# matchylabs/matchy

Measured on AMD Instinct MI355X. Metric: log GB/s scanned (matchy match hot path, 100K IoCs), higher is better.
Workload: dtype u8

## Files before the change

include/matchy_amd.h:

```cpp
#ifndef MATCHY_AMD_H
#define MATCHY_AMD_H

#include <stdbool.h>
#include <stddef.h>
#include <stdint.h>

#ifdef __cplusplus
extern "C" {
#endif

#define MATCHY_SUCCESS 0
#define MATCHY_ERROR_FILE_NOT_FOUND -1
#define MATCHY_ERROR_INVALID_FORMAT -2
#define MATCHY_ERROR_CORRUPT_DATA -3
#define MATCHY_ERROR_OUT_OF_MEMORY -4
#define MATCHY_ERROR_INVALID_PARAM -5
#define MATCHY_ERROR_IO -6

#define MATCHY_EXTRACT_DOMAINS (1 << 0)
#define MATCHY_EXTRACT_EMAILS (1 << 1)
#define MATCHY_EXTRACT_IPV4 (1 << 2)
#define MATCHY_EXTRACT_IPV6 (1 << 3)
#define MATCHY_EXTRACT_HASHES (1 << 4)
#define MATCHY_EXTRACT_BITCOIN (1 << 5)
// ... 290 lines not shown
typedef struct matchy_gz_piece_t {
    uint64_t start_bit, end_bit;
    uint32_t member;
    uint32_t produced, out_pos;
    uint32_t flags;
} matchy_gz_piece_t;
#define MATCHY_PIECE_HAS_START 1u
#define MATCHY_PIECE_LIVE 2u
#define MATCHY_PIECE_HANDED_OVER 4u
int32_t matchy_scanner_set_gz_pieces(matchy_scanner_t *scanner, uint32_t piece_bytes);
uint32_t matchy_scanner_get_gz_pieces(const matchy_scanner_t *scanner);
int32_t matchy_scan_result_gz_pieces(const matchy_scan_result_t *result, const matchy_gz_piece_t **pieces, size_t *n, const uint32_t **first_piece);
void matchy_scanner_get_gz_pieces_timing(const matchy_scanner_t *scanner, float out_ms[6]);
typedef struct matchy_gz_stream_state_t { uint64_t text_bytes; uint32_t crc, bit, history_len; uint8_t history[32768]; } matchy_gz_stream_state_t;
typedef struct matchy_gz_stream_window_t {
    const matchy_gz_stream_state_t *state;
    const uint8_t *carry; uint32_t carry_len, carry_cap, text_cap, flags;
} matchy_gz_stream_window_t;
#define MATCHY_STREAM_FIRST 1u
#define MATCHY_STREAM_FILE_END 2u
#define MATCHY_STREAM_OK 0
#define MATCHY_STREAM_NO_LINE_END 1
#define MATCHY_STREAM_NO_PROGRESS 2
#define MATCHY_STREAM_FAILED 3
int32_t matchy_scanner_scan_gz_stream(matchy_scanner_t *scanner, const uint8_t *packed, size_t packed_len, const matchy_gz_stream_window_t *window,
                                      uint32_t fetch_mode, bool want_text, matchy_scan_result_t *result);
int32_t matchy_scan_result_gz_stream(const matchy_scan_result_t *result, int32_t *status, int32_t *gz_status, uint64_t *consumed_bits, uint32_t *text_len,
                                     bool *ended, const matchy_gz_stream_state_t **state_out, const uint8_t **carry, size_t *carry_len);
#define MATCHY_STREAM_PASSES 8
void matchy_scanner_get_gz_stream_timing(const matchy_scanner_t *scanner, float out_ms[MATCHY_STREAM_PASSES]);
void matchy_scanner_set_profile(matchy_scanner_t *scanner, bool enabled);
void matchy_scanner_set_slices(matchy_scanner_t *scanner, int32_t slices);
int32_t matchy_scanner_last_slices(const matchy_scanner_t *scanner);
void matchy_scanner_get_timing(const matchy_scanner_t *scanner, float out_ms[5]);
char *matchy_amd_query_json(const matchy_t *db, const char *query, int32_t *found);
matchy_extractor_t *matchy_amd_extractor_create(uint32_t flags, uint32_t min_domain_labels);
void matchy_amd_extractor_set_unique(matchy_extractor_t *extractor, bool enabled);
bool matchy_amd_extractor_unique(const matchy_extractor_t *extractor);
void matchy_amd_extractor_reset_unique(matchy_extractor_t *extractor);
uint64_t matchy_amd_extractor_unique_count(const matchy_extractor_t *extractor);
const char *matchy_amd_last_error(void);
int32_t matchy_amd_ac_dfa_states(const matchy_t *db);
int32_t matchy_amd_suffix_filter(const matchy_t *db);
void *matchy_amd_pinned_alloc(size_t bytes);
void matchy_amd_pinned_free(void *ptr);
int32_t matchy_amd_host_register(const void *ptr, size_t bytes);
void matchy_amd_host_unregister(const void *ptr);
int32_t matchy_amd_device_count(void);
int32_t matchy_amd_device_numa_node(int32_t device);
int32_t matchy_amd_bind_thread_to_device(int32_t device);
int32_t matchy_amd_unbind_thread(void);
int32_t matchy_amd_numa_cpus(const char *sysfs_root, const char *pci_bus_id, int32_t *out_cpus, size_t cap);

typedef struct matchy_multi_scanner_t matchy_multi_scanner_t;
typedef struct matchy_multi_batch_t {
  size_t seq;
  int32_t status;
  matchy_scan_result_t result;
  const uint8_t *data;
  size_t len;
  void *tag;
  void *payload;
  size_t worker;
} matchy_multi_batch_t;
typedef struct matchy_multi_totals_t { uint64_t batches, bytes, lines, candidates, matches; } matchy_multi_totals_t;
typedef void *(*matchy_multi_batch_fn)(void *user, size_t worker, matchy_scanner_t *scanner, const matchy_scan_result_t *result,
// ... 66 lines not shown
```

matchy_amd/__init__.py:

```python
import ctypes as C
import os
import json
from pathlib import Path

from . import build as _build

__all__ = ["DatabaseBuilder", "Database", "Extractor", "Scanner", "lib", "ITEM_TYPE_NAMES", "EXTRACT_ALL", "last_error"]

PKG = Path(__file__).resolve().parent
LIB_PATH = PKG / "lib" / "libmatchy_amd.so"

ITEM_TYPE_NAMES = ["Domain", "Email", "IPv4", "IPv6", "MD5", "SHA1", "SHA256", "SHA384", "SHA512", "Bitcoin", "Ethereum", "Monero"]
EXTRACT_DOMAINS, EXTRACT_EMAILS, EXTRACT_IPV4, EXTRACT_IPV6 = 1, 2, 4, 8
EXTRACT_HASHES, EXTRACT_BITCOIN, EXTRACT_ETHEREUM, EXTRACT_MONERO = 16, 32, 64, 128
EXTRACT_ALL = 255

EXPORTED_SYMBOLS = [
    "matchy_builder_new", "matchy_builder_set_case_insensitive", "matchy_builder_add", "matchy_builder_set_description",
    "matchy_builder_save", "matchy_builder_build", "matchy_builder_free", "matchy_init_open_options",
    "matchy_open_with_options", "matchy_open", "matchy_open_buffer", "matchy_close", "matchy_query", "matchy_query_into",
    "matchy_free_result", "matchy_free_string", "matchy_result_to_json", "matchy_version", "matchy_format",
    "matchy_has_ip_data", "matchy_has_string_data", "matchy_has_literal_data", "matchy_has_glob_data", "matchy_metadata",
    "matchy_get_pattern_string", "matchy_pattern_count", "matchy_extractor_create", "matchy_extractor_extract_chunk",
    "matchy_matches_free", "matchy_extractor_free", "matchy_item_type_name", "matchy_scanner_create", "matchy_scanner_free",
    "matchy_scanner_scan", "matchy_scanner_scan_device", "matchy_scan_result_free", "matchy_scan_hit_to_json",
    "matchy_scanner_set_profile", "matchy_scanner_get_timing", "matchy_amd_last_error", "matchy_builder_set_build_epoch",
    "matchy_get_stats", "matchy_clear_cache", "matchy_has_pattern_data", "matchy_result_get_entry", "matchy_aget_value",
    "matchy_get_entry_data_list", "matchy_free_entry_data_list", "matchy_validate", "matchy_builder_set_schema",
    "matchy_amd_query_json", "matchy_amd_extractor_create", "matchy_amd_device_count", "matchy_scanner_submit_device",
    "matchy_scanner_wait", "matchy_scanner_set_slices", "matchy_scanner_last_slices", "matchy_scan_result_on_device",
    "matchy_amd_ac_dfa_states", "matchy_amd_suffix_filter", "matchy_amd_pinned_alloc", "matchy_amd_pinned_free",
    "matchy_amd_host_register", "matchy_amd_host_unregister",
    "matchy_amd_device_numa_node", "matchy_amd_bind_thread_to_device", "matchy_amd_numa_cpus",
    "matchy_multi_scanner_create", "matchy_multi_scanner_free", "matchy_multi_scanner_workers", "matchy_multi_scanner_worker_scanner",
    "matchy_multi_scanner_set_batch_hook", "matchy_multi_scanner_submit", "matchy_multi_scanner_next", "matchy_multi_scanner_scan",
    "matchy_multi_scanner_pending", "matchy_multi_scanner_max_pending", "matchy_multi_scanner_submit_near", "matchy_multi_scanner_worker_numa",
    "matchy_amd_unbind_thread",
    "matchy_multi_scanner_scan_file", "matchy_scan_result_to_ndjson",
    "matchy_scanner_set_line_context", "matchy_scanner_line_context", "matchy_scan_result_lines", "matchy_multi_scanner_set_line_context",
    "matchy_scan_result_to_ndjson_lines", "matchy_scanner_get_line_timing",
    "matchy_amd_extractor_set_unique", "matchy_amd_extractor_unique", "matchy_amd_extractor_reset_unique", "matchy_amd_extractor_unique_count",
    "matchy_scanner_set_tally", "matchy_scanner_tally", "matchy_scanner_reset_tally", "matchy_scanner_tally_top",
    "matchy_multi_scanner_set_tally", "matchy_multi_scanner_tally_top", "matchy_multi_scanner_reset_tally", "matchy_tally_free",
    "matchy_scanner_set_segments", "matchy_scan_result_segments", "matchy_scan_result_to_ndjson_segments",
    "matchy_multi_scanner_submit_segments", "matchy_scanner_get_segment_timing",
    "matchy_scanner_scan_gz", "matchy_scan_result_gz", "matchy_scanner_get_gz_timing", "matchy_multi_scanner_submit_gz",
    "matchy_scanner_scan_gz_files", "matchy_scan_result_gz_files", "matchy_multi_scanner_submit_gz_files",
    "matchy_scanner_scan_gz_window", "matchy_scan_result_gz_window", "matchy_multi_scanner_submit_gz_window", "matchy_scanner_get_gz_window_timing",
    "matchy_scanner_set_gz_pieces", "matchy_scanner_get_gz_pieces", "matchy_scan_result_gz_pieces", "matchy_scanner_get_gz_pieces_timing",
    "matchy_multi_scanner_set_gz_pieces",
    "matchy_scanner_scan_gz_stream", "matchy_scan_result_gz_stream", "matchy_scanner_get_gz_stream_timing", "matchy_multi_scanner_submit_gz_stream",
    "matchy_scanner_set_hit_lines", "matchy_scanner_hit_lines", "matchy_scan_result_hit_lines", "matchy_scanner_get_hit_lines_timing",
    "matchy_multi_scanner_set_hit_lines",
    "matchy_scanner_set_render", "matchy_scan_result_ndjson", "matchy_scanner_get_render_timing", "matchy_scanner_get_render_counters",
    "matchy_multi_scanner_set_render",
    "matchy_scanner_set_whole_lines", "matchy_scanner_whole_lines", "matchy_scanner_get_whole_lines_counters",
    "matchy_scanner_get_whole_lines_timing", "matchy_multi_scanner_set_whole_lines",
    "matchy_scanner_scan_utf16", "matchy_scan_result_utf16", "matchy_scanner_get_utf16_timing", "matchy_amd_utf16_geometry",
    "matchy_multi_scanner_submit_utf16",
]

UTF16_LE, UTF16_BE = 0, 1

# ... 224 lines not shown
        "matchy_has_literal_data": (C.c_bool, [vp]),
        "matchy_has_glob_data": (C.c_bool, [vp]),
        "matchy_metadata": (vp, [vp]),
        "matchy_get_pattern_string": (vp, [vp, C.c_uint32]),
        "matchy_pattern_count": (C.c_size_t, [vp]),
        "matchy_extractor_create": (vp, [C.c_uint32]),
        "matchy_amd_extractor_create": (vp, [C.c_uint32, C.c_uint32]),
        "matchy_extractor_extract_chunk": (C.c_int32, [vp, cp, C.c_size_t, C.POINTER(_Matches)]),
        "matchy_matches_free": (None, [C.POINTER(_Matches)]),
        "matchy_extractor_free": (None, [vp]),
        "matchy_amd_extractor_set_unique": (None, [vp, C.c_bool]),
        "matchy_amd_extractor_unique": (C.c_bool, [vp]),
        "matchy_amd_extractor_reset_unique": (None, [vp]),
        "matchy_amd_extractor_unique_count": (C.c_uint64, [vp]),
        "matchy_item_type_name": (cp, [C.c_uint8]),
        "matchy_scanner_create": (vp, [vp, C.c_uint32, C.c_int32]),
        "matchy_scanner_free": (None, [vp]),
        "matchy_scanner_scan": (C.c_int32, [vp, vp, C.c_size_t, C.POINTER(_ScanResult)]),
        "matchy_scanner_scan_device": (C.c_int32, [vp, vp, C.c_size_t, vp, C.c_uint32, C.POINTER(_ScanResult)]),
        "matchy_scanner_submit_device": (C.c_int32, [vp, vp, C.c_size_t, vp, C.c_uint32]),
        "matchy_scanner_wait": (C.c_int32, [vp, C.POINTER(_ScanResult)]),
        "matchy_scan_result_free": (None, [C.POINTER(_ScanResult)]),
        "matchy_scan_hit_to_json": (vp, [vp, C.POINTER(_ScanResult), C.c_size_t, cp, cp]),
        "matchy_scan_result_to_ndjson": (C.c_int32, [vp, C.POINTER(_ScanResult), cp, cp, C.POINTER(vp), C.POINTER(C.c_size_t)]),
        "matchy_scanner_set_profile": (None, [vp, C.c_bool]),
        "matchy_amd_ac_dfa_states": (C.c_int32, [vp]),
        "matchy_amd_suffix_filter": (C.c_int32, [vp]),
        "matchy_amd_pinned_alloc": (vp, [C.c_size_t]),
        "matchy_amd_pinned_free": (None, [vp]),
        "matchy_amd_host_register": (C.c_int32, [vp, C.c_size_t]),
        "matchy_amd_host_unregister": (None, [vp]),
        "matchy_scanner_set_slices": (None, [vp, C.c_int32]),
        "matchy_scanner_last_slices": (C.c_int32, [vp]),
        "matchy_scan_result_on_device": (C.c_bool, [C.POINTER(_ScanResult)]),
        "matchy_scanner_get_timing": (None, [vp, C.POINTER(C.c_float)]),
        "matchy_amd_last_error": (cp, []),
        "matchy_get_stats": (None, [vp, C.POINTER(_Stats)]),
        "matchy_clear_cache": (None, [vp]),
        "matchy_has_pattern_data": (C.c_bool, [vp]),
        "matchy_result_get_entry": (C.c_int32, [C.POINTER(_Result), C.POINTER(_Entry)]),
        "matchy_aget_value": (C.c_int32, [C.POINTER(_Entry), C.POINTER(_EntryData), C.POINTER(cp)]),
        "matchy_get_entry_data_list": (C.c_int32, [C.POINTER(_Entry), C.POINTER(C.POINTER(_EntryDataList))]),
        "matchy_free_entry_data_list": (None, [C.POINTER(_EntryDataList)]),
        "matchy_validate": (C.c_int32, [cp, C.c_int32, C.POINTER(vp)]),
        "matchy_builder_set_schema": (C.c_int32, [vp, cp]),
        "matchy_amd_device_count": (C.c_int32, []),
        "matchy_amd_device_numa_node": (C.c_int32, [C.c_int32]),
        "matchy_amd_bind_thread_to_device": (C.c_int32, [C.c_int32]),
        "matchy_amd_numa_cpus": (C.c_int32, [cp, cp, C.POINTER(C.c_int32), C.c_size_t]),
        "matchy_multi_scanner_create": (vp, [vp, C.c_uint32, C.POINTER(C.c_int32), C.c_size_t]),
        "matchy_multi_scanner_free": (None, [vp]),
        "matchy_multi_scanner_workers": (C.c_size_t, [vp]),
        "matchy_multi_scanner_worker_scanner": (vp, [vp, C.c_size_t]),
        "matchy_multi_scanner_submit": (C.c_int32, [vp, vp, C.c_size_t, vp, vp]),
        "matchy_multi_scanner_next": (C.c_int32, [vp, C.POINTER(_MultiBatch)]),
        "matchy_multi_scanner_submit_near": (C.c_int32, [vp, vp, C.c_size_t, vp, vp, C.c_int32]),
        "matchy_multi_scanner_worker_numa": (C.c_int32, [vp, C.c_size_t, C.POINTER(C.c_int32), C.POINTER(C.c_int32)]),
        "matchy_multi_scanner_pending": (C.c_size_t, [vp]),
        "matchy_multi_scanner_max_pending": (C.c_size_t, [vp]),
        "matchy_amd_unbind_thread": (C.c_int32, []),
        "matchy_multi_scanner_scan": (C.c_int32, [vp, vp, C.c_size_t, C.c_size_t, C.POINTER(_ScanResult)]),
        "matchy_multi_scanner_scan_file": (C.c_int32, [vp, cp, C.c_size_t, _MULTI_ORDERED_FN, vp, C.POINTER(_MultiTotals)]),
        "matchy_scanner_set_line_context": (None, [vp, C.c_bool]),
        "matchy_scanner_line_context": (C.c_bool, [vp]),
        "matchy_scan_result_lines": (C.c_int32, [C.POINTER(_ScanResult), C.POINTER(vp), C.POINTER(vp), C.POINTER(C.c_uint64)]),
        "matchy_multi_scanner_set_line_context": (None, [vp, C.c_bool]),
# ... 810 lines not shown
    def gz_pieces_timing_ms(self):
        out = (C.c_float * 6)()
        lib().matchy_scanner_get_gz_pieces_timing(self._h, out)
        return dict(find=out[0], count=out[1], chain=out[2], symbols=out[3], resolve=out[4], handover=out[5])

    def gz_window_timing_ms(self):
        out = (C.c_float * 4)()
        lib().matchy_scanner_get_gz_window_timing(self._h, out)
        return dict(inflate=out[0], crc=out[1], seal=out[2], tail=out[3])

    def gz_timing_ms(self):
        out = (C.c_float * 3)()
        lib().matchy_scanner_get_gz_timing(self._h, out)
        return dict(inflate=out[0], crc=out[1], seal=out[2])

    def set_tally(self, on=True):
        lib().matchy_scanner_set_tally(self._h, bool(on))

    def tally_enabled(self) -> bool:
        return bool(lib().matchy_scanner_tally(self._h))

    def reset_tally(self):
        lib().matchy_scanner_reset_tally(self._h)

    def tally(self, limit=0):
        return _read_tally(lib().matchy_scanner_tally_top, self._h, limit, "matchy_scanner_tally_top")

    def set_slices(self, n: int):
        lib().matchy_scanner_set_slices(self._h, n)

    def last_slices(self) -> int:
        return lib().matchy_scanner_last_slices(self._h)

    def timing_ms(self):
        out = (C.c_float * 5)()
        lib().matchy_scanner_get_timing(self._h, out)
        return dict(anchor=out[0], validate=out[1], rare=out[2], lookup=out[3], total=out[4])

    def close(self):
        if self._h:
            lib().matchy_scanner_free(self._h)
            self._h = None

    def __del__(self):
        try:
            self.close()
        except Exception:
            pass


def _gz_pack(blobs, out_lens=None):
    table = (_GzMember * len(blobs))()
    pos = 0
    for i, b in enumerate(blobs):
        table[i].offset, table[i].len = pos, len(b)
        table[i].out_len = int(out_lens[i]) if out_lens is not None and out_lens[i] else 0
        pos += len(b)
    return b"".join(bytes(b) for b in blobs), table


def _gz_pack_files(blobs):
    table = (_GzFile * len(blobs))()
    pos = 0
    for i, b in enumerate(blobs):
        table[i].offset, table[i].len = pos, len(b)
        pos += len(b)
# ... 208 lines not shown
```

matchy_amd/csrc/capi.cpp:

```cpp
#include "../../include/matchy_amd.h"

#include <algorithm>
#include <atomic>
#include <cstddef>
#include <cstdio>
#include <cstdlib>
#include <chrono>
#include <cstring>
#include <list>
#include <memory>
#include <mutex>
#include <string>
#include <unordered_map>
#include <unordered_set>
#include <vector>

#include "capi_internal.h"
#include "db_builder.h"
#include "db_image.h"
#include "engine.h"
#include "gz_stream.h"
#include "host_lookup.h"
#include "inflate_core.h"
#include "ndjson_host.h"
// ... 888 lines not shown
        for (size_t i = 0; i < in->items.size(); ++i) in->items[i].value = in->values[i].c_str();
        out->items = in->items.data(); out->count = in->items.size(); out->_internal = in;
        return MATCHY_SUCCESS;
    } catch (const HipError& ex) { set_error(ex.what); return MATCHY_ERROR_IO; }
    catch (const std::exception& ex) { set_error(ex.what()); return MATCHY_ERROR_IO; }
}
void matchy_matches_free(matchy_matches_t* m) {
    if (!m) return;
    delete reinterpret_cast<MatchesInternal*>(m->_internal);
    m->items = nullptr; m->count = 0; m->_internal = nullptr;
}

matchy_scanner_t* matchy_scanner_create(const matchy_t* dbc, uint32_t extract_flags, int32_t device) {
    if (!dbc || device < 0) return nullptr;
    Db* db = const_cast<Db*>(reinterpret_cast<const Db*>(dbc));
    try {
        if (extract_flags == 0) {
            if (db->img->has_ip) extract_flags |= EX_IPV4 | EX_IPV6;
            if (db->img->has_literal || db->img->has_glob) extract_flags |= EX_DOMAINS | EX_EMAILS | EX_HASHES | EX_BITCOIN | EX_ETHEREUM | EX_MONERO;
        }
        std::shared_ptr<DeviceDb> ddb;
        { std::lock_guard<std::mutex> lk(db->mu); ddb = db->device_db(device); }
        auto s = std::make_unique<ScannerH>();
        s->db = db;
        s->sc = std::make_unique<Scanner>(db->img, ddb, extract_flags, 2);
        return reinterpret_cast<matchy_scanner_t*>(s.release());
    } catch (const HipError& e) { set_error(e.what); return nullptr; }
    catch (const std::exception& e) { set_error(e.what()); return nullptr; }
}
void matchy_scanner_free(matchy_scanner_t* s) { delete reinterpret_cast<ScannerH*>(s); }
void matchy_scanner_set_profile(matchy_scanner_t* s, bool on) { if (s) reinterpret_cast<ScannerH*>(s)->sc->set_profile(on); }
void matchy_scanner_set_slices(matchy_scanner_t* s, int32_t n) { if (s) reinterpret_cast<ScannerH*>(s)->sc->set_slices(n); }
int32_t matchy_scanner_last_slices(const matchy_scanner_t* s) { return s ? reinterpret_cast<const ScannerH*>(s)->sc->last_slice_count() : 0; }
void matchy_scanner_set_line_context(matchy_scanner_t* s, bool on) { if (s) reinterpret_cast<ScannerH*>(s)->sc->set_line_context(on); }
bool matchy_scanner_line_context(const matchy_scanner_t* s) { return s && reinterpret_cast<const ScannerH*>(s)->sc->line_context(); }
void matchy_scanner_get_line_timing(const matchy_scanner_t* s, float out[3]) {
    if (s && out) reinterpret_cast<const ScannerH*>(s)->sc->line_timing(out);
}
int32_t matchy_scan_result_lines(const matchy_scan_result_t* r, const matchy_scan_line_t** lines, const matchy_scan_line_t** ip4_lines, uint64_t* lines_with_matches) {
    if (!r) return MATCHY_ERROR_INVALID_PARAM;
    const ScanResultInternal* in = reinterpret_cast<const ScanResultInternal*>(r->_internal);
    if (!in || !in->has_lines) { set_error("matchy_scan_result_lines: the result was produced with line context off"); return MATCHY_ERROR_INVALID_PARAM; }
    if (lines) *lines = in->lines;
    if (ip4_lines) *ip4_lines = in->ip4_lines;
    if (lines_with_matches) *lines_with_matches = in->lines_with_matches;
    return MATCHY_SUCCESS;
}

void matchy_scanner_set_hit_lines(matchy_scanner_t* s, bool on) { if (s) reinterpret_cast<ScannerH*>(s)->sc->set_hit_lines(on); }
bool matchy_scanner_hit_lines(const matchy_scanner_t* s) { return s && reinterpret_cast<const ScannerH*>(s)->sc->hit_lines(); }
int32_t matchy_scan_result_hit_lines(const matchy_scan_result_t* r, matchy_scan_hit_lines_t* out) {
    if (!r || !out) return MATCHY_ERROR_INVALID_PARAM;
    const ScanResultInternal* in = reinterpret_cast<const ScanResultInternal*>(r->_internal);
    if (!in || !in->has_hit_lines) { set_error("matchy_scan_result_hit_lines: the result was produced with hit lines off"); return MATCHY_ERROR_INVALID_PARAM; }
    *out = in->hit_lines;
    return MATCHY_SUCCESS;
}
void matchy_scanner_get_hit_lines_timing(const matchy_scanner_t* s, float out[3]) {
    if (s && out) reinterpret_cast<const ScannerH*>(s)->sc->hit_lines_timing(out);
}

void matchy_scanner_set_whole_lines(matchy_scanner_t* s, bool on) { if (s) reinterpret_cast<ScannerH*>(s)->sc->set_whole_lines(on); }
bool matchy_scanner_whole_lines(const matchy_scanner_t* s) { return s && reinterpret_cast<const ScannerH*>(s)->sc->whole_lines(); }
void matchy_scanner_get_whole_lines_counters(const matchy_scanner_t* s, uint64_t out[4]) {
    if (s && out) reinterpret_cast<const ScannerH*>(s)->sc->whole_lines_counters(out);
}
// ... 458 lines not shown
```

matchy_amd/csrc/domain_prefilter.h:

```cpp
#pragma once
#include <cstdint>

#include "hashes.h"

namespace mxy {

struct ByteMasks { uint64_t dc, dot, dash, high; };
struct ByteMasks32 { uint32_t dc, dot, dash, high; };
MXY_HD ByteMasks32 domain_masks32(uint32_t x) {
    constexpr uint32_t H = 0x80808080u, L7 = 0x7F7F7F7Fu;
    const uint32_t t = x & L7, l = t | 0x20202020u;
    const uint32_t dig = (t + 0x50505050u) & ~(t + 0x46464646u);
    const uint32_t alp = (l + 0x1F1F1F1Fu) & ~(l + 0x05050505u);
    const uint32_t ndot = (t ^ 0x2E2E2E2Eu) + L7, ndash = (t ^ 0x2D2D2D2Du) + L7;
    ByteMasks32 m;
    m.high = x & H;
    m.dot = ~ndot & ~x & H;
    m.dash = ~ndash & ~x & H;
    m.dc = (((dig | alp) & ~x) | m.dot | m.dash | m.high) & H;
    return m;
}
MXY_HD ByteMasks domain_masks(uint64_t x) {
    const ByteMasks32 lo = domain_masks32((uint32_t)x), hi = domain_masks32((uint32_t)(x >> 32));
    ByteMasks m;
    m.dc = (uint64_t)lo.dc | ((uint64_t)hi.dc << 32);
    m.dot = (uint64_t)lo.dot | ((uint64_t)hi.dot << 32);
    m.dash = (uint64_t)lo.dash | ((uint64_t)hi.dash << 32);
    m.high = (uint64_t)lo.high | ((uint64_t)hi.high << 32);
    return m;
}

constexpr uint32_t TLD_PREFILTER_BITS = 1u << 14;

template <class Boundary>
MXY_HD bool label_window_keep(uint32_t lo, uint32_t hi, const uint32_t* filter, Boundary is_boundary) {
    constexpr uint32_t H = 0x80808080u;
    const ByteMasks32 ml = domain_masks32(lo), mh = domain_masks32(hi);
    const uint32_t nl = ~ml.dc & H, nh = ~mh.dc & H;
    const uint32_t el = (nl & (0u - nl)) >> 7, eh = nl ? 0u : (nh & (0u - nh)) >> 7;
    const uint32_t bl = el - 1u, bh = nl ? 0u : eh - 1u;
    const bool full = (nl | nh) == 0;
    const uint32_t at = nl ? (uint32_t)__builtin_ctz(nl) - 7u : (uint32_t)__builtin_ctz(nh | 0x80000000u) - 7u;
    const uint32_t stop = ((nl ? lo : hi) >> at) & 0xFFu;
    const uint32_t h8 = tld_hash8(lo & bl, hi & bh);
    const uint32_t b1 = h8 & (TLD_PREFILTER_BITS - 1), b2 = (h8 >> 14) & (TLD_PREFILTER_BITS - 1);
    const uint32_t in_filter = (filter[b1 >> 5] >> (b1 & 31)) & (filter[b2 >> 5] >> (b2 & 31)) & 1u;
    return (((ml.dot & bl) | (mh.dot & bh)) == 0) & (full | is_boundary(stop)) & (in_filter != 0);
}

template <class Slot>
inline bool prefilter_add_label(uint32_t* filter, Slot* pfx, const uint8_t* last, size_t ll) {
    uint8_t k8[8] = {0};
    for (size_t k = 0; k < ll && k < 8; ++k) k8[k] = last[k];
    const uint32_t lo = k8[0] | (uint32_t)k8[1] << 8 | (uint32_t)k8[2] << 16 | (uint32_t)k8[3] << 24;
    const uint32_t hi = k8[4] | (uint32_t)k8[5] << 8 | (uint32_t)k8[6] << 16 | (uint32_t)k8[7] << 24;
    const uint32_t h8 = tld_hash8(lo, hi);
    const uint32_t b1 = h8 & (TLD_PREFILTER_BITS - 1), b2 = (h8 >> 14) & (TLD_PREFILTER_BITS - 1);
    filter[b1 >> 5] |= 1u << (b1 & 31);
    filter[b2 >> 5] |= 1u << (b2 & 31);
    return ll >= 8 && tld_pfx_insert(pfx, lo, hi);
}

}
```

matchy_amd/csrc/engine.cpp:

```cpp
#include "engine.h"
#include "batch_reader.h"
#include "distinct.h"
#include "render_core.h"
#include "tally.h"
#include "unicode_lower.h"

#include <dlfcn.h>

#include <algorithm>
#include <chrono>
#include <cstdio>
#include <cstdlib>
#include <cstring>
#include <stdexcept>
#include <unordered_set>

#include "domain_prefilter.h"
#include "hashes.h"

namespace mxy {

void check_launch(const char* kernel) {
    const hipError_t e = hipGetLastError();
    if (e != hipSuccess) throw HipError{std::string("launch of ") + kernel + ": " + hipGetErrorString(e)};
// ... 494 lines not shown
    ensure_final(work_[0].hits.n, work_[0].ids.n);
}

static_assert(sizeof(FinalHit) == ResultLayout::REC_BYTES, "result_layout.h lays out FinalHit records");

namespace {
struct ResultArrays { FinalHit* recs; uint32_t* ids; long long* offs; };
ResultArrays arrays_of(uint8_t* block, const ResultLayout& l) {
    return {(FinalHit*)block, (uint32_t*)(block + l.ids_offset()), (long long*)(block + l.offs_offset())};
}
}

void Scanner::ensure_mirror(uint32_t recs, uint32_t ids) {
    if (mirror_.p && mirror_layout_.recs_cap >= recs && mirror_layout_.ids_cap >= ids) return;
    const ResultLayout want{std::max<size_t>(recs, mirror_layout_.recs_cap), std::max<size_t>(ids, mirror_layout_.ids_cap)};
    mirror_layout_ = ResultLayout{};
    mirror_.alloc(want.bytes());
    mirror_layout_ = want;
}

namespace {
void grid_multipliers(bool filter_ac, int (&gm)[3]) {
    static const int occ_a = anchor_blocks_per_cu(), occ_v = validate_blocks_per_cu(false), occ_v_ac = validate_blocks_per_cu(true);
    gm[0] = occ_a; gm[1] = std::min(filter_ac ? occ_v_ac : occ_v, 4); gm[2] = 2;
    for (int& m : gm) m = std::max(1, std::min(m, 64));
}
}

int Scanner::grid_for(uint32_t n_hint, uint32_t per_wg, int dflt, int max_per_cu) const {
    const uint64_t want = ((uint64_t)n_hint + per_wg - 1) / per_wg;
    return (int)std::max<uint64_t>((uint64_t)dflt, std::min<uint64_t>(want, (uint64_t)n_cu_ * (uint64_t)max_per_cu));
}

namespace {
size_t grown_list(uint32_t n) { return (size_t)n + n / 4 + 1024; }
void point_at(TokParams& t, const DevBuf<Candidate>& l, uint32_t* n) { t.cands = l.p; t.cand_cap = (uint32_t)l.n; t.n_cand = n; }
void point_at(LookupParams& p, const DevBuf<Candidate>& l, const uint32_t* n) { p.cands = l.p; p.cand_cap = (uint32_t)l.n; p.n_in = n; }
}

void Scanner::slice_params(int sl, const ScanRequest& rq, uint32_t lo, uint32_t hi, SliceLaunch& L) {
    const uint8_t* dptr = rq.ptr;
    const uint32_t len = rq.len;
    const bool lookup = rq.lookup;
    Work& w = work_[sl];
    ScanCounters* ctr = counters_.p + sl;
    TokParams& tp = L.tp;
    tp = TokParams{};
    tp.log = dptr; tp.len = len; tp.flags = flags_; tp.min_labels = min_labels_;
    tp.filter_v4 = lookup ? 1u : 0u;
    const bool ac_ok = ddb_->view.has_glob && ddb_->view.dfa && ddb_->view.wild_count == 0;
    tp.filter_ac = (lookup && ac_ok) ? 1u : 0u;
    tp.filter_lit = (lookup && (!ddb_->view.has_glob || ac_ok)) ? 1u : 0u;
    if (const char* dbg = getenv("MATCHY_AMD_DEBUG")) tp.debug = (uint32_t)atoi(dbg);
    point_at(tp, w.cands, &ctr->n_cand);
    tp.cands_a = w.cands_a.p; tp.cand_a_cap = (uint32_t)w.cands_a.n;
    tp.cand_chunk = (lookup && ddb_->view.ip_bm24_permille <= 250) ? 64u : 1024u;
    tp.rare = w.rare.p; tp.rare_cap = (uint32_t)w.rare.n;
    tp.rare_dom = w.rare_dom.p; tp.rare_dom_cap = (uint32_t)w.rare_dom.n;
    tp.vmode = 7u;
    tp.tok = w.tok.p; tp.tok_cap = (uint32_t)w.tok.n;
    tp.heavy = w.heavy.p; tp.heavy_cap = (uint32_t)w.heavy.n;
    tp.dom_list = w.dom_list.p; tp.dom_cap = (uint32_t)w.dom_slots;
    tp.counters = ctr;
    grid_multipliers(tp.filter_ac != 0, L.gm);
    {
        const uint64_t waves = (uint64_t)n_cu_ * L.gm[0] * 4;
// ... 248 lines not shown
    launch_validate_misc(t1, view, grid_for(rare_own ? hint_.n_rare : std::max(hint_.n_rare, hint_.n_tok), 1024, std::max(1, n_cu_ / 2), rare_own ? RARE_WGS_PER_CU : 8), aux2_stream_);
    uint32_t chains = 0;
    if (L.split_misc) {
        LookupParams lm = L.lm;
        if (rare_own || !rare_possible()) { lm.arrive_chain = 1; lm.arrive = ctr; ++chains; }
        launch_lookup(lm, view, grid_for(hint_.n_cand_m, 512, std::max(1, n_cu_ / 2), 4), aux2_stream_);
    }
    if (rare_possible()) {
        TokParams tr = t1;
        tr.vmode = tp.vmode;
        if (L.split_misc) point_at(tr, w.cands_r, &ctr->n_cand_r);
        hipStream_t rs = rare_own ? aux_stream_ : aux2_stream_;
        if (rare_own && !tok_aside) MXY_HIP(hipStreamWaitEvent(aux_stream_, ev_v1_, 0));
        launch_rare(tr, view, grid_for(hint_.n_heavy, 128, n_cu_ * 4, 16), rs);
        if (L.split_misc) {
            LookupParams lr = L.lr;
            lr.arrive_chain = rare_own ? 2u : 1u; lr.arrive = ctr; ++chains;
            launch_lookup(lr, view, grid_for(hint_.n_cand_r, 512, std::max(1, n_cu_ / 8), 4), rs);
        }
    }
    if (!L.split_misc) MXY_HIP(hipEventRecord(ev_join2_, aux2_stream_));
    launch_validate_dom(tp, view, n_cu_ * L.gm[1], stream);
    TokParams t2 = tp;
    t2.vmode = 2u;
    if (L.split_misc) {
        ensure_dom_stream();
        MXY_HIP(hipEventRecord(ev_dom_, stream));
        MXY_HIP(hipStreamWaitEvent(dom_stream_, ev_dom_, 0));
        LookupParams lpm = L.lp;
        lpm.arrive_chain = 3; lpm.arrive = ctr; ++chains;
        launch_lookup(lpm, view, grid_for(hint_.n_cand, 512, n_cu_, 4), dom_stream_);
        expect_chains_ = chains;
        point_at(t2, w.cands_d, &ctr->n_cand_d);
        launch_validate_misc(t2, view, grid_for(hint_.n_rare_dom, 512, n_cu_, RARE_DOM_WGS_PER_CU), stream);
        launch_lookup(L.ld, view, grid_for(hint_.n_cand_d, 512, std::max(1, n_cu_ / 8), 4), stream);
    } else {
        const bool v2_aside = early_glob_ && !L.ip_pass;
        if (early_glob_) {
            ensure_dom_stream();
            MXY_HIP(hipEventRecord(ev_dom_, stream));
            MXY_HIP(hipStreamWaitEvent(dom_stream_, ev_dom_, 0));
            LookupParams lg = L.lp;
            lg.glob_work = w.glob_work_d.p; lg.glob_work_cap = (uint32_t)w.glob_work_d.n;
            lg.n_work = &ctr->n_glob_work_d;
            lg.arrive_chain = 3; lg.arrive = ctr; ++chains;
            launch_lookup_early_glob(lg, view, n_cu_ * L.gm[2], dom_stream_);
            if (v2_aside) {
                MXY_HIP(hipStreamWaitEvent(aux_stream_, ev_dom_, 0));
                point_at(t2, w.cands_d, &ctr->n_cand_d);
                launch_validate_misc(t2, view, grid_for(hint_.n_rare_dom, 512, n_cu_, 8), aux_stream_);
                LookupParams ld = L.ld;
                ld.arrive_chain = 2; ld.arrive = ctr; ++chains;
                launch_lookup(ld, view, grid_for(hint_.n_cand_d, 512, std::max(2, n_cu_ / 8), 4), aux_stream_);
            }
            expect_chains_ = chains;
        }
        if (!v2_aside) launch_validate_misc(t2, view, grid_for(hint_.n_rare_dom, 512, n_cu_, RARE_DOM_WGS_PER_CU), stream);
        MXY_HIP(hipStreamWaitEvent(stream, ev_join2_, 0));
        if (last_.lookup) launch_lookup(L.lp, view, n_cu_ * L.gm[2], stream);
    }
    if (L.ip_pass) MXY_HIP(hipStreamWaitEvent(stream, ev_join_, 0));
}

void Scanner::launch_one_stream(hipStream_t stream) {
    const SliceLaunch& L = launch_[0];
    const TokParams& tp = L.tp;
    const DevDb& view = ddb_->view;
    launch_anchor(tp, view, L.grid_anchor, stream);
// ... 166 lines not shown
            if (trace) fprintf(stderr, "[matchy_amd] %u candidates to the spill pass\n", n_spill);
            continue;
        }
        if (trace) fprintf(stderr, "[matchy_amd] work buffers overflow (attempt %d): regrow and rescan:%s\n", attempt, over_names.c_str());
        if (single_) throw HipError{"lookup_one: work buffers overflow"};
        if (attempt >= MAX_REGROWS) throw HipError{"scan: work buffers still overflow after regrowing"};
        ++attempt;
        size_t recs = 0, ids = 0;
        for (int k = 0; k < ns; ++k) {
            each_list(work_[k], host_slices_.p[k], [](const char*, size_t cap, size_t need, auto&& grow) { if (need > cap) grow(); });
            recs += work_[k].hits.n; ids += work_[k].ids.n;
        }
        if (final_.n < recs || c.n_final > final_.n) final_.alloc(std::max<size_t>(recs, grown(c.n_final)));
        if (final_ids_.n < recs + ids || c.n_final_ids > final_ids_.n) {
            const size_t want = std::max<size_t>(recs + ids, grown(c.n_final_ids));
            final_ids_.alloc(want); final_offs_.alloc(want);
        }
        if (compact_ && c.n_c4 > c4_.n) c4_.alloc(grown(c.n_c4));
        scan_device(last_, stream);
    }
}

void Scanner::report_counters(ScanOutput& out, bool trace) {
    const int ns = n_slices_;
    {
        ListHint hh;
        for (int k = 0; k < ns; ++k) {
            const ScanCounters& q = host_slices_.p[k];
            hh.n_tok = std::max(hh.n_tok, q.n_tok); hh.n_rare = std::max(hh.n_rare, q.n_rare); hh.n_rare_dom = std::max(hh.n_rare_dom, q.n_rare_dom);
            hh.n_heavy = std::max(hh.n_heavy, q.n_heavy); hh.n_cand = std::max(hh.n_cand, q.n_cand); hh.n_cand_m = std::max(hh.n_cand_m, q.n_cand_m);
            hh.n_cand_r = std::max(hh.n_cand_r, q.n_cand_r); hh.n_cand_d = std::max(hh.n_cand_d, q.n_cand_d);
            hh.n_dom = std::max(hh.n_dom, q.n_dom);
        }
        hint_ = hh;
    }
    const ScanCounters& c = host_counters_;
    if (c.error & 1) throw HipError{"scan: a candidate matches more than 65535 glob patterns (the hit record counts pattern ids in 16 bits)"};
    if (c.error & 4) throw HipError{"scan: a candidate is longer than 16 MiB (24-bit length field)"};
    if (trace) {
        ScanCounters t = host_slices_.p[0];
        for (int k = 1; k < ns; ++k) {
            const ScanCounters& s = host_slices_.p[k];
            t.n_dom += s.n_dom; t.n_rare += s.n_rare; t.n_rare_dom += s.n_rare_dom; t.n_tok += s.n_tok; t.n_heavy += s.n_heavy; t.n_cand_a += s.n_cand_a;
            t.n_cand += s.n_cand; t.n_hits += s.n_hits; t.n_ids += s.n_ids; t.n_glob_work += s.n_glob_work;
        }
        fprintf(stderr, "[matchy_amd] slices=%d lines=%llu n_dom=%u n_rare=%u+%u n_tok=%u n_heavy=%u n_cand=%u+%u (true %u) n_hits=%u (true %u) n_ids=%u glob_work=%u final=%u\n",
                ns, c.lines, t.n_dom, t.n_rare, t.n_rare_dom, t.n_tok, t.n_heavy, t.n_cand_a, t.n_cand, c.cand_true, t.n_hits, c.hits_true, t.n_ids, t.n_glob_work, c.n_final);
    }
    out.lines = c.lines; out.n_cand = single_ ? c.n_cand : c.cand_true;
    out.n_hits = !last_.lookup ? 0 : (single_ ? c.hits_true : c.n_final + (compact_ ? c.n_c4 : 0u));
    if (profile_) {
        MXY_HIP(hipEventElapsedTime(&timing_.anchor_ms, ev_[0], ev_[1]));
        if (last_forked_) {
            MXY_HIP(hipEventElapsedTime(&timing_.validate_ms, ev_[1], ev_[4]));
            timing_.rare_ms = 0; timing_.lookup_ms = 0;
        } else {
            MXY_HIP(hipEventElapsedTime(&timing_.validate_ms, ev_[1], ev_[2]));
            MXY_HIP(hipEventElapsedTime(&timing_.rare_ms, ev_[2], ev_[3]));
            MXY_HIP(hipEventElapsedTime(&timing_.lookup_ms, ev_[3], ev_[4]));
        }
        MXY_HIP(hipEventElapsedTime(&timing_.total_ms, ev_[0], ev_[4]));
        timing_.slices = ns;
    }
    if (last_.whole_lines && wl_) {
        const WholeLineCounters& h = *wl_->host.p;
        wl_->last[0] = h.queries; wl_->last[1] = h.address(); wl_->last[2] = h.string(); wl_->last[3] = h.invalid_utf8;
        out.n_cand = h.address() + h.string();
// ... 539 lines not shown
```

matchy_amd/csrc/engine.h:

```cpp
#pragma once
#include <hip/hip_runtime.h>

#include <memory>
#include <mutex>
#include <string>
#include <vector>

#include "db_image.h"
#include "hip_owners.h"
#include "hit_lines.h"
#include "inflate.h"
#include "line_index.h"
#include "render.h"
#include "result_layout.h"
#include "scan_types.h"
#include "segments.h"
#include "utf16.h"
#include "whole_lines.h"

namespace mxy {

int anchor_blocks_per_cu();
int validate_blocks_per_cu(bool ac);
void launch_anchor(const TokParams& p, const DevDb& db, int grid, hipStream_t stream);
// ... 166 lines not shown
    void gz_queue_results(bool want_text);
    GzInflate::Result gz_finish();
    void gz_timing(float out_ms[3]) const { for (int k = 0; k < 3; ++k) out_ms[k] = 0; if (gz_) gz_->timing(out_ms); }
    void set_gz_pieces(uint32_t piece_bytes) { gz_piece_bytes_ = piece_bytes; }
    uint32_t gz_pieces() const { return gz_piece_bytes_; }
    void gz_pieces_timing(float out_ms[6]) const { for (int k = 0; k < 6; ++k) out_ms[k] = 0; if (gz_) gz_->pieces_timing(out_ms); }
    void gz_stream_timing(float out_ms[GZ_STREAM_PASSES]) const { for (int k = 0; k < GZ_STREAM_PASSES; ++k) out_ms[k] = 0; if (gz_) gz_->stream_timing(out_ms); }
    void gz_window_timing(float out_ms[4]) const { gz_timing(out_ms); out_ms[3] = gz_ ? gz_->tail_ms() : 0; }
    GzBatch utf16_transcode(const uint8_t* src, size_t len, uint32_t byte_order);
    void utf16_queue_text(bool want_text);
    Utf16Transcode::Result utf16_finish();
    void utf16_timing(float out_ms[3]) const { for (int k = 0; k < 3; ++k) out_ms[k] = 0; if (utf16_) utf16_->timing(out_ms); }
    void set_whole_lines(bool on) { whole_lines_ = on; }
    bool whole_lines() const { return whole_lines_; }
    void arm_whole_lines(ScanRequest& rq, bool gz = false);
    void whole_lines_counters(uint64_t out[4]) const { for (int k = 0; k < 4; ++k) out[k] = wl_ ? wl_->last[k] : 0; }
    void whole_lines_timing(float out_ms[3]) const { for (int k = 0; k < 3; ++k) out_ms[k] = wl_ ? wl_->ms[k] : 0; }
    void set_unique(bool on);
    bool unique() const { return unique_; }
    void reset_unique();
    uint64_t unique_count() const;
    void set_tally(bool on);
    bool tally() const { return tally_on_; }
    void reset_tally();
    const HitTally* hit_tally() const { return tally_.get(); }
    void tally_top(size_t limit, std::vector<TallyEntry>& out);
    void lookup_one(const std::string& text, Candidate c, ScanOutput& out);
    void scan_host(const uint8_t* data, size_t len, bool lookup, bool want_cands, ScanOutput& out, std::vector<uint64_t>* cand_bases,
                   std::vector<FinalHit>* fin, std::vector<uint32_t>* fin_ids, std::vector<long long>* fin_offs, std::vector<LineRec>* fin_lines = nullptr);
    void set_profile(bool on) { profile_ = on; }
    void set_slices(int n) { slices_ = n < 0 ? 0 : n; }
    int slices() const { return slices_; }
    int last_slice_count() const { return n_slices_; }
    const ScanTiming& timing() const { return timing_; }
    uint32_t flags() const { return flags_; }
    int device() const { return ddb_->device; }
    const DbImage& image() const { return *img_; }

    static constexpr int MAX_SLICES = 8;
    static constexpr uint32_t SPILL_BLOCKS = 16;

private:
    struct Work {
        DevBuf<Candidate> cands, cands_a;
        DevBuf<Candidate> cands_m, cands_r, cands_d;
        DevBuf<RareAnchor> rare, rare_dom, tok, heavy;
        DevBuf<uint32_t> dom_list;
        size_t dom_slots = 0;
        DevBuf<Hit> hits;
        DevBuf<uint32_t> ids, glob_work;
        DevBuf<uint32_t> glob_work_d;
        DevBuf<uint32_t> spill;
        void ensure(uint32_t len);
    };
    Work work_[MAX_SLICES];
    int n_slices_ = 1;
    int slices_ = 0;
    void ensure_capacity(uint32_t len);
    void ensure_final(size_t recs, size_t ids);
    struct SliceLaunch {
        TokParams tp;
        LookupParams lp, la, lm, lr, ld;
        bool split_misc = false;
        int gm[3] = {1, 1, 1};
        int grid_anchor = 1, ip_grid = 1;
        bool ip_pass = false, ip_dense = false;
    };
    SliceLaunch launch_[MAX_SLICES];
    void slice_params(int sl, const ScanRequest& rq, uint32_t lo, uint32_t hi, SliceLaunch& L);
    int plan_slices(uint32_t len, int want, uint32_t (&cuts)[MAX_SLICES + 1]);
    void setup_spill(int sl, LookupParams& lp);
    void launch_sliced(int ns, hipStream_t stream);
    void launch_forked(hipStream_t stream);
    void launch_one_stream(hipStream_t stream);
    void launch_whole_lines(const ScanRequest& rq, hipStream_t stream);
    void ensure_dom_stream();
    bool rare_possible() const { return (flags_ & (EX_HASHES | EX_BITCOIN | EX_ETHEREUM | EX_MONERO)) != 0; }
    void settle_counters(bool trace, hipStream_t stream);
    void report_counters(ScanOutput& out, bool trace);
    const FinalHit* queue_record_copies(ScanOutput& out, bool want_cands, HitMode hit_mode, bool sorted, hipStream_t stream);
    void queue_post_passes(ScanOutput& out, const FinalHit* dev_recs, bool want_cands, HitMode hit_mode, bool trace, hipStream_t stream);
    void finish_fetch(ScanOutput& out, bool want_cands, HitMode hit_mode, hipStream_t stream);
    template <class F> void each_list(Work& w, const ScanCounters& s, F&& f);
    bool spill_done_ = false;
    bool early_glob_ = false;
    uint32_t expect_chains_ = 0;
    struct ListHint { uint32_t n_tok = 0, n_rare = 0, n_rare_dom = 0, n_heavy = 0, n_cand = 0, n_cand_m = 0, n_cand_r = 0, n_cand_d = 0, n_dom = 0; } hint_;
    uint32_t dom_preset_ = 0;
    uint32_t dom_want_ = 0;
    int grid_for(uint32_t n_hint, uint32_t per_wg, int dflt, int max_per_cu) const;
    bool counters_clean_ = false;
    ScanRequest last_;
    std::shared_ptr<const DbImage> img_;
    std::shared_ptr<DeviceDb> ddb_;
    Stream host_stream_;
    uint32_t flags_, min_labels_;
    Stream aux_stream_;
    Event ev_fork_, ev_join_;
    Stream aux2_stream_;
    Event ev_join2_;
    Stream dom_stream_;
    Event ev_anchor_[MAX_SLICES], ev_misc_[MAX_SLICES];
    Event ev_join3_, ev_dom_, ev_v1_;
    DevBuf<FinalHit> final_;
    DevBuf<uint32_t> final_ids_;
    DevBuf<long long> final_offs_;
    DevBuf<unsigned long long> sort_keys_;
    DevBuf<uint32_t> sort_vals_;
    DevBuf<uint8_t> sort_tmp_;
    DevBuf<FinalHit> final_sorted_;
    DevBuf<ScanCounters> counters_;
    bool line_ctx_ = false;
    std::unique_ptr<LineContext> lines_;
    bool hit_lines_on_ = false;
    std::unique_ptr<HitLines> hit_lines_;
    std::unique_ptr<SegmentPass> segments_;
    std::unique_ptr<RenderParams> render_pending_;
    std::unique_ptr<NdjsonRender> render_;
    std::unique_ptr<GzInflate> gz_;
    uint32_t gz_piece_bytes_ = 0;
    std::unique_ptr<Utf16Transcode> utf16_;
    struct HostPin {
        uintptr_t a = 0, b = 0;
        void release();
        ~HostPin() { release(); }
    } utf16_pin_;
    template <class Launch> GzBatch gz_pass(Launch&& launch);
    struct WholeLines {
        DevBuf<uint32_t> counts, chunks, prefix, ends;
        DevBuf<uint8_t> invalid;
        DevBuf<WholeLineCounters> ctr;
        PinnedBuf<WholeLineCounters> host;
        uint64_t last[4] = {0, 0, 0, 0};
        float ms[3] = {0, 0, 0};
    };
    bool whole_lines_ = false;
    std::unique_ptr<WholeLines> wl_;
    bool unique_ = false;
    std::unique_ptr<DistinctSet> distinct_;
    bool tally_on_ = false;
    std::unique_ptr<HitTally> tally_;
    DevBuf<uint32_t> spill_scratch_;
    DevBuf<uint8_t> staging_;
    PinnedBuf<uint8_t> mirror_;
    ResultLayout mirror_layout_;
    bool mirror_used_ = false;
    void ensure_mirror(uint32_t recs, uint32_t ids);
    DevBuf<uint2> c4_;
    PinnedBuf<uint2> mirror_c4_, pinned_c4_;
    bool compact_ = false;
    PinnedBuf<uint8_t> pinned_;
    void ensure_pinned(size_t bytes) { pinned_.ensure(bytes, bytes / 4 + (1 << 16)); }
    ScanCounters host_counters_{};
    PinnedBuf<ScanCounters> host_slices_;
    bool last_forked_ = false;
    bool single_ = false;
    bool profile_ = false;
    Event ev_[5];
    ScanTiming timing_;
    int n_cu_ = 256;
};

}
```

matchy_amd/csrc/k_anchor.hip:

```cpp
#include "anchor_planes.h"
#include "device_shared.h"

namespace mxy {

constexpr int AW = 4;
constexpr int PRIO_BULK = 0, PRIO_CHAIN = 1, PRIO_DRAIN = 2;
constexpr uint32_t BLK_BYTES = AB_BLOCK;
constexpr uint32_t QCAP = 128;
constexpr uint32_t RAW_BYTES = 8192;
static_assert(SEG_ALIGN % RAW_BYTES == 0 && RAW_BYTES % BLK_BYTES == 0 && RAW_BYTES >= 3 * BLK_BYTES, "window wraps on block edges inside a segment");

constexpr uint32_t RAW_MIRROR = 64;
template <int N>
__device__ __forceinline__ void raw_read(const uint32_t* raw32, uint32_t a, uint32_t (&out)[N]) {
    static_assert(4 * (N + 1) <= RAW_MIRROR + 4, "read runs past the mirrored bytes");
    const uint32_t* q = raw32 + ((a & (RAW_BYTES - 1)) >> 2);
    const uint32_t sh = a & 3;
    uint32_t w[N + 1];
#pragma unroll
    for (int i = 0; i <= N; ++i) w[i] = q[i];
#pragma unroll
    for (int i = 0; i < N; ++i) out[i] = __builtin_amdgcn_alignbyte(w[i + 1], w[i], sh);
}

// ... 283 lines not shown
        pd.ok = true;
        pd.n_valid += 1;
        pd.word = p.filter_v4 ? cx.bm24[a >> 13] : 0xFFFFFFFFu;
    }
    __builtin_amdgcn_wave_barrier();
    __builtin_amdgcn_s_setprio(PRIO_CHAIN);
}

__device__ __forceinline__ void drain_dom(uint32_t* ring, uint32_t& head, uint32_t& tail, uint32_t n, bool final, const WaveCtx& cx,
                                          DomWriter& dw) {
    const uint32_t lane = lane_id();
    const TokParams& p = *cx.p;
    __builtin_amdgcn_s_setprio(PRIO_DRAIN);
    __builtin_amdgcn_wave_barrier();
    uint32_t ent = 0;
    const bool have = lane < n;
    if (have) ent = ring[(head + lane) & (QCAP - 1)];
    const uint32_t j = have ? anchor_pos(ent) : 0xFFFFFFFFu;
    head += n;
    const bool later = have && !final && j + 8 > cx.res_hi;
    const uint64_t rm = __ballot(later);
    if (rm) {
        __builtin_amdgcn_wave_barrier();
        if (later) ring[(tail + mbcnt64(rm)) & (QCAP - 1)] = ent;
        tail += (uint32_t)__popcll(rm);
    }
#ifdef MXY_ANCHOR_DEBUG
    if (p.debug & 2) { __builtin_amdgcn_s_setprio(PRIO_CHAIN); return; }
#endif
    const bool go = have && !later;
    const bool have_ctx = go && j >= cx.res_lo + 24 && j + 8 <= cx.res_hi;
    uint32_t ctx[8];
    raw_read<8>(cx.raw32, j - 24, ctx);
    const bool k = label_window_keep(ctx[6], ctx[7], cx.bloom, [](uint32_t b) { return d_is_boundary(b); });
    const bool keep = have_ctx ? k : go;
    const uint32_t slot = dw.reserve(keep, p.dom_list, p.dom_cap, [] { return &cold_tok()->counters->n_dom; },
                                     [] { const uint32_t st = cold_tok()->dom_static; return st ? (blockIdx.x * 4u + (threadIdx.x >> 6)) * st : 0xFFFFFFFFu; },
                                     [] { return cold_tok()->dom_chunk; });
    if (slot != 0xFFFFFFFFu) {
        uint32_t* rec = p.dom_list + dom_plane_index(slot, 0);
        rec[0] = have_ctx ? j : (j | 0x80000000u);
#pragma unroll
        for (int k = 0; k < 8; ++k) rec[(1 + k) * DOM_TILE] = ctx[k];
    }
    __builtin_amdgcn_wave_barrier();
    __builtin_amdgcn_s_setprio(PRIO_CHAIN);
}

__host__ __device__ inline bool anchor_tl_wide(const DevDb& db) {
    uint32_t outside = 0;
    for (int k = 0; k < 8; ++k) {
        const uint32_t allowed = k >= 4 ? 0xFFFFFFFFu : (k == 3 ? 0x07FFFFFEu : 0u);
        outside |= db.tld_first[k] & ~allowed;
    }
    return outside != 0;
}

constexpr int DPP_WAVE_SHL1 = 0x130, DPP_WAVE_SHR1 = 0x138, DPP_WAVE_ROR1 = 0x13C;
__device__ __forceinline__ uint32_t plane_prev_dword(uint32_t P, uint32_t& carry) {
    const uint32_t s63 = (uint32_t)__builtin_amdgcn_readlane((int)P, 63);
    const uint32_t fix0 = ((s63 << 1) & 0xFEFEFEFEu) | ((carry >> 7) & 0x01010101u);
    carry = s63;
    return (uint32_t)__builtin_amdgcn_update_dpp((int)fix0, (int)P, DPP_WAVE_SHR1, 0xF, 0xF, false);
}
__device__ __forceinline__ uint32_t plane_next_dword(uint32_t P, uint32_t ahead) {
    const uint32_t s0 = (uint32_t)__builtin_amdgcn_readlane((int)P, 0);
    const uint32_t fix63 = ((s0 >> 1) & 0x7F7F7F7Fu) | ahead;
    return (uint32_t)__builtin_amdgcn_update_dpp((int)fix63, (int)P, DPP_WAVE_SHL1, 0xF, 0xF, false);
}
__device__ __forceinline__ uint32_t wave_incl_scan_add(uint32_t v) {
    v += (uint32_t)__builtin_amdgcn_update_dpp(0, (int)v, 0x111, 0xF, 0xF, true);
    v += (uint32_t)__builtin_amdgcn_update_dpp(0, (int)v, 0x112, 0xF, 0xF, true);
    v += (uint32_t)__builtin_amdgcn_update_dpp(0, (int)v, 0x114, 0xF, 0xF, true);
    v += (uint32_t)__builtin_amdgcn_update_dpp(0, (int)v, 0x118, 0xF, 0xF, true);
// ... 361 lines not shown
```

Before: 2385.

## Read boundary anchor context from the log and size near-empty grids to one workgroup

Anchors that sit near the edge of the resident raw window now rebuild their label context straight from the global log, byte by byte, padding past the end with spaces. This lets the bloom keep-filter run on every anchor instead of passing edge anchors through unfiltered with a flag bit, so fewer domain records go downstream. Separately, once list-size hints are known, the rare-domain validate and domain lookup launches shrink their grid to one workgroup when the hinted list fits in a single workgroup. The change also adds a host API that reports per-list counters. The fallback path costs slow per-lane global byte loads, and the single-workgroup sizing depends on hints taken from earlier scans.

```diff
diff --git a/include/matchy_amd.h b/include/matchy_amd.h
--- a/include/matchy_amd.h
+++ b/include/matchy_amd.h
@@ -346,6 +346,7 @@
 void matchy_scanner_set_profile(matchy_scanner_t *scanner, bool enabled);
 void matchy_scanner_set_slices(matchy_scanner_t *scanner, int32_t slices);
 int32_t matchy_scanner_last_slices(const matchy_scanner_t *scanner);
+void matchy_scanner_get_list_counts(const matchy_scanner_t *scanner, uint64_t out[8]);
 void matchy_scanner_get_timing(const matchy_scanner_t *scanner, float out_ms[5]);
 char *matchy_amd_query_json(const matchy_t *db, const char *query, int32_t *found);
 matchy_extractor_t *matchy_amd_extractor_create(uint32_t flags, uint32_t min_domain_labels);
diff --git a/matchy_amd/__init__.py b/matchy_amd/__init__.py
--- a/matchy_amd/__init__.py
+++ b/matchy_amd/__init__.py
@@ -28,7 +28,7 @@
     "matchy_get_stats", "matchy_clear_cache", "matchy_has_pattern_data", "matchy_result_get_entry", "matchy_aget_value",
     "matchy_get_entry_data_list", "matchy_free_entry_data_list", "matchy_validate", "matchy_builder_set_schema",
     "matchy_amd_query_json", "matchy_amd_extractor_create", "matchy_amd_device_count", "matchy_scanner_submit_device",
-    "matchy_scanner_wait", "matchy_scanner_set_slices", "matchy_scanner_last_slices", "matchy_scan_result_on_device",
+    "matchy_scanner_wait", "matchy_scanner_set_slices", "matchy_scanner_last_slices", "matchy_scanner_get_list_counts", "matchy_scan_result_on_device",
     "matchy_amd_ac_dfa_states", "matchy_amd_suffix_filter", "matchy_amd_pinned_alloc", "matchy_amd_pinned_free",
     "matchy_amd_host_register", "matchy_amd_host_unregister",
     "matchy_amd_device_numa_node", "matchy_amd_bind_thread_to_device", "matchy_amd_numa_cpus",
@@ -319,6 +319,7 @@
         "matchy_amd_host_unregister": (None, [vp]),
         "matchy_scanner_set_slices": (None, [vp, C.c_int32]),
         "matchy_scanner_last_slices": (C.c_int32, [vp]),
+        "matchy_scanner_get_list_counts": (None, [vp, C.POINTER(C.c_uint64)]),
         "matchy_scan_result_on_device": (C.c_bool, [C.POINTER(_ScanResult)]),
         "matchy_scanner_get_timing": (None, [vp, C.POINTER(C.c_float)]),
         "matchy_amd_last_error": (cp, []),
@@ -1195,6 +1196,12 @@
     def last_slices(self) -> int:
         return lib().matchy_scanner_last_slices(self._h)
 
+    def list_counts(self):
+        out = (C.c_uint64 * 8)()
+        lib().matchy_scanner_get_list_counts(self._h, out)
+        names = ("n_dom", "n_rare", "n_rare_dom", "n_tok", "n_heavy", "n_cand_a", "n_cand", "n_hits")
+        return {n: int(out[k]) for k, n in enumerate(names)}
+
     def timing_ms(self):
         out = (C.c_float * 5)()
         lib().matchy_scanner_get_timing(self._h, out)
diff --git a/matchy_amd/csrc/capi.cpp b/matchy_amd/csrc/capi.cpp
--- a/matchy_amd/csrc/capi.cpp
+++ b/matchy_amd/csrc/capi.cpp
@@ -944,6 +944,10 @@
 void matchy_scanner_set_profile(matchy_scanner_t* s, bool on) { if (s) reinterpret_cast<ScannerH*>(s)->sc->set_profile(on); }
 void matchy_scanner_set_slices(matchy_scanner_t* s, int32_t n) { if (s) reinterpret_cast<ScannerH*>(s)->sc->set_slices(n); }
 int32_t matchy_scanner_last_slices(const matchy_scanner_t* s) { return s ? reinterpret_cast<const ScannerH*>(s)->sc->last_slice_count() : 0; }
+void matchy_scanner_get_list_counts(const matchy_scanner_t* s, uint64_t out[8]) {
+    static_assert(Scanner::LIST_COUNTS == 8, "matchy_amd.h documents eight counters");
+    if (s && out) reinterpret_cast<const ScannerH*>(s)->sc->list_counts(out);
+}
 void matchy_scanner_set_line_context(matchy_scanner_t* s, bool on) { if (s) reinterpret_cast<ScannerH*>(s)->sc->set_line_context(on); }
 bool matchy_scanner_line_context(const matchy_scanner_t* s) { return s && reinterpret_cast<const ScannerH*>(s)->sc->line_context(); }
 void matchy_scanner_get_line_timing(const matchy_scanner_t* s, float out[3]) {
diff --git a/matchy_amd/csrc/domain_prefilter.h b/matchy_amd/csrc/domain_prefilter.h
--- a/matchy_amd/csrc/domain_prefilter.h
+++ b/matchy_amd/csrc/domain_prefilter.h
@@ -48,6 +48,16 @@
     return (((ml.dot & bl) | (mh.dot & bh)) == 0) & (full | is_boundary(stop)) & (in_filter != 0);
 }
 
+MXY_HD uint32_t label_context_dword(const uint8_t* log, uint32_t len, uint32_t j, uint32_t k) {
+    const uint32_t pos0 = j - 24u + 4u * k;
+    uint32_t x = 0;
+    for (uint32_t b = 0; b < 4; ++b) {
+        const uint32_t pos = pos0 + b;
+        x |= (pos < len ? (uint32_t)log[pos] : (uint32_t)' ') << (8 * b);
+    }
+    return x;
+}
+
 template <class Slot>
 inline bool prefilter_add_label(uint32_t* filter, Slot* pfx, const uint8_t* last, size_t ll) {
     uint8_t k8[8] = {0};
diff --git a/matchy_amd/csrc/engine.cpp b/matchy_amd/csrc/engine.cpp
--- a/matchy_amd/csrc/engine.cpp
+++ b/matchy_amd/csrc/engine.cpp
@@ -550,6 +550,8 @@
     return (int)std::max<uint64_t>((uint64_t)dflt, std::min<uint64_t>(want, (uint64_t)n_cu_ * (uint64_t)max_per_cu));
 }
 
+bool Scanner::near_empty(uint32_t n_hint, uint32_t per_wg) const { return hint_.known && n_hint <= per_wg; }
+
 namespace {
 size_t grown_list(uint32_t n) { return (size_t)n + n / 4 + 1024; }
 void point_at(TokParams& t, const DevBuf<Candidate>& l, uint32_t* n) { t.cands = l.p; t.cand_cap = (uint32_t)l.n; t.n_cand = n; }
@@ -864,8 +866,8 @@
         launch_lookup(lpm, view, grid_for(hint_.n_cand, 512, n_cu_, 4), dom_stream_);
         expect_chains_ = chains;
         point_at(t2, w.cands_d, &ctr->n_cand_d);
-        launch_validate_misc(t2, view, grid_for(hint_.n_rare_dom, 512, n_cu_, RARE_DOM_WGS_PER_CU), stream);
-        launch_lookup(L.ld, view, grid_for(hint_.n_cand_d, 512, std::max(1, n_cu_ / 8), 4), stream);
+        launch_validate_misc(t2, view, grid_for(hint_.n_rare_dom, 512, near_empty(hint_.n_rare_dom, 512) ? 1 : n_cu_, RARE_DOM_WGS_PER_CU), stream);
+        launch_lookup(L.ld, view, grid_for(hint_.n_cand_d, 512, near_empty(hint_.n_cand_d, 512) ? 1 : std::max(1, n_cu_ / 8), 4), stream);
     } else {
         const bool v2_aside = early_glob_ && !L.ip_pass;
         if (early_glob_) {
@@ -1098,7 +1100,14 @@
             hh.n_cand_r = std::max(hh.n_cand_r, q.n_cand_r); hh.n_cand_d = std::max(hh.n_cand_d, q.n_cand_d);
             hh.n_dom = std::max(hh.n_dom, q.n_dom);
         }
+        hh.known = true;
         hint_ = hh;
+        for (uint64_t& v : list_counts_) v = 0;
+        for (int k = 0; k < ns; ++k) {
+            const ScanCounters& q = host_slices_.p[k];
+            const uint32_t v[LIST_COUNTS] = {q.n_dom, q.n_rare, q.n_rare_dom, q.n_tok, q.n_heavy, q.n_cand_a, q.n_cand, q.n_hits};
+            for (int i = 0; i < LIST_COUNTS; ++i) list_counts_[i] += v[i];
+        }
     }
     const ScanCounters& c = host_counters_;
     if (c.error & 1) throw HipError{"scan: a candidate matches more than 65535 glob patterns (the hit record counts pattern ids in 16 bits)"};
diff --git a/matchy_amd/csrc/engine.h b/matchy_amd/csrc/engine.h
--- a/matchy_amd/csrc/engine.h
+++ b/matchy_amd/csrc/engine.h
@@ -222,6 +222,8 @@
     void set_slices(int n) { slices_ = n < 0 ? 0 : n; }
     int slices() const { return slices_; }
     int last_slice_count() const { return n_slices_; }
+    static constexpr int LIST_COUNTS = 8;
+    void list_counts(uint64_t out[LIST_COUNTS]) const { for (int k = 0; k < LIST_COUNTS; ++k) out[k] = list_counts_[k]; }
     const ScanTiming& timing() const { return timing_; }
     uint32_t flags() const { return flags_; }
     int device() const { return ddb_->device; }
@@ -275,10 +277,11 @@
     bool spill_done_ = false;
     bool early_glob_ = false;
     uint32_t expect_chains_ = 0;
-    struct ListHint { uint32_t n_tok = 0, n_rare = 0, n_rare_dom = 0, n_heavy = 0, n_cand = 0, n_cand_m = 0, n_cand_r = 0, n_cand_d = 0, n_dom = 0; } hint_;
+    struct ListHint { uint32_t n_tok = 0, n_rare = 0, n_rare_dom = 0, n_heavy = 0, n_cand = 0, n_cand_m = 0, n_cand_r = 0, n_cand_d = 0, n_dom = 0; bool known = false; } hint_;
     uint32_t dom_preset_ = 0;
     uint32_t dom_want_ = 0;
     int grid_for(uint32_t n_hint, uint32_t per_wg, int dflt, int max_per_cu) const;
+    bool near_empty(uint32_t n_hint, uint32_t per_wg) const;
     bool counters_clean_ = false;
     ScanRequest last_;
     std::shared_ptr<const DbImage> img_;
@@ -342,6 +345,7 @@
     PinnedBuf<uint8_t> pinned_;
     void ensure_pinned(size_t bytes) { pinned_.ensure(bytes, bytes / 4 + (1 << 16)); }
     ScanCounters host_counters_{};
+    uint64_t list_counts_[LIST_COUNTS] = {};
     PinnedBuf<ScanCounters> host_slices_;
     bool last_forked_ = false;
     bool single_ = false;
diff --git a/matchy_amd/csrc/k_anchor.hip b/matchy_amd/csrc/k_anchor.hip
--- a/matchy_amd/csrc/k_anchor.hip
+++ b/matchy_amd/csrc/k_anchor.hip
@@ -339,14 +339,26 @@
     const bool have_ctx = go && j >= cx.res_lo + 24 && j + 8 <= cx.res_hi;
     uint32_t ctx[8];
     raw_read<8>(cx.raw32, j - 24, ctx);
-    const bool k = label_window_keep(ctx[6], ctx[7], cx.bloom, [](uint32_t b) { return d_is_boundary(b); });
-    const bool keep = have_ctx ? k : go;
+    if (__ballot(go && !have_ctx)) {
+        if (go && !have_ctx) {
+            const ColdTok kp = cold_tok();
+            const uint8_t* const log = kp->log;
+            const uint32_t len = kp->len;
+#pragma unroll 1
+            for (uint32_t q = 0; q < 8; ++q) {
+                const uint32_t x = label_context_dword(log, len, j, q);
+#pragma unroll
+                for (uint32_t r = 0; r < 8; ++r) ctx[r] = r == q ? x : ctx[r];
+            }
+        }
+    }
+    const bool keep = go && label_window_keep(ctx[6], ctx[7], cx.bloom, [](uint32_t b) { return d_is_boundary(b); });
     const uint32_t slot = dw.reserve(keep, p.dom_list, p.dom_cap, [] { return &cold_tok()->counters->n_dom; },
                                      [] { const uint32_t st = cold_tok()->dom_static; return st ? (blockIdx.x * 4u + (threadIdx.x >> 6)) * st : 0xFFFFFFFFu; },
                                      [] { return cold_tok()->dom_chunk; });
     if (slot != 0xFFFFFFFFu) {
         uint32_t* rec = p.dom_list + dom_plane_index(slot, 0);
-        rec[0] = have_ctx ? j : (j | 0x80000000u);
+        rec[0] = j;
 #pragma unroll
         for (int k = 0; k < 8; ++k) rec[(1 + k) * DOM_TILE] = ctx[k];
     }
```

Result: no change. 2386, median of 3 (+0.0%).
